# AndrewCullacino/handwritten-chinese-ocr-samples

Hardware: AMD Instinct MI355X
Metric: text-lines/sec (1x128x2000 synth) greedy decode (higher is better)
Workload: dtype f16 (f32 accumulate); 1 GPU; BASELINE configs[1]: 64 x 1x128x2000 uint8 lines, random-init hctr checkpoint (C=7358), forward + greedy CTC decode, labels to host; global_lines=64, lines_per_gpu=64, width=2000, classes=7358, checkpoint=random, parallelism=batch-shard x1

## Files before the change

### handwritten-chinese-ocr-samples_amd/csrc/engine.cpp

```cpp
#include "../../include/hctr_hip.h"
#include "kernels.h"

#include <algorithm>
#include <cfloat>
#include <cmath>
#include <cstdarg>
#include <cstdio>
#include <cstring>
#include <map>
#include <new>
#include <string>
#include <vector>

using namespace hctr;

namespace {

constexpr int kImgH = 128;
constexpr int kFeat = 2048;
constexpr double kBnEps = 1e-5;
constexpr int kStagePlanes[4] = {128, 256, 512, 512};
constexpr int kStageBlocks[4] = {2, 4, 5, 1};
constexpr int kStageH[5] = {128, 64, 32, 16, 8};
constexpr int64_t kDefaultMaxCols = 131072;
// ... 25 lines not shown
};

struct Workspace {
    int B = 0, W = 0, Wa = 0;
    void* img = nullptr;
    int32_t* widths = nullptr;
    half_t* s0 = nullptr;
    half_t* x[5] = {};
    half_t* p[5][3] = {};
    half_t* headin = nullptr;
    float* logits = nullptr;
    float* se_part = nullptr;
    float* se_scale = nullptr;
    float* se_border = nullptr;
    float* se_mean = nullptr;
    int32_t* se_counter = nullptr;
    int32_t* colidx = nullptr;
    float* amax_val = nullptr;
    int32_t* amax_idx = nullptr;
    int32_t* labels = nullptr;
    int32_t* lengths = nullptr;
    float* psum = nullptr;
    float* blank_logit = nullptr;
    float* row_thr = nullptr;
    int32_t* emit_cnt = nullptr;
    int32_t* emit_list = nullptr;
    double* esum = nullptr;
    int32_t* overflow = nullptr;
    int32_t* bm_idx = nullptr;
    float* bm_lp = nullptr;
    float* bm_bl = nullptr;
    float* bm_st = nullptr;
    int32_t* bm_cnt = nullptr;
    int32_t* tile_ctrs = nullptr;
    float* amax_val2 = nullptr;
    float* amax_abs = nullptr;
    float* col_margin = nullptr;
    float* col_abs = nullptr;
    float* line_guard = nullptr;
    int features = 0;
    bool split = false;
    bool aliased = false;
};

enum WsFeature { WS_S0 = 1, WS_LOGITS = 2, WS_BEAM = 4, WS_GUARD = 8 };

struct WeightSet {
    float* stem_w = nullptr;
    float* stem_b = nullptr;
    ConvW conv0_2;
    std::vector<BlockW> blocks[4];
    ConvW stage_conv[4];
    ConvW head;
    bool built = false;
};

struct ProfEntry {
    std::string name;
    hipEvent_t e0, e1;
};

}

struct hctr_ctx {
    int device = 0;
    int num_classes = 0;
    int cpad = 0;
    hipStream_t stream = nullptr;
    std::string err;
    std::map<std::string, HostTensor> host;
    bool finalized = false;
    WeightSet wset[2];
    const WeightSet& wts() const { return wset[split ? 1 : 0]; }
    std::vector<void*> wallocs;
    Workspace ws;
    char* arena = nullptr;
    size_t arena_cap = 0;
    int ws_sticky = 0;
    int64_t arena_reallocs = 0, ws_recarves = 0;
    int ws_alias = -1;
    size_t ws_dedicated_max = (size_t)16 << 30;
    int64_t max_cols = kDefaultMaxCols;
    bool big_tiles = true;
    int halo_mode = 2;
    int mode = 0;
    bool split = false;
    int x3_mask = 31;
    int out_class = 8;
    double guard_rel = 0.01, guard_abs = 0.05;
    std::vector<float> g_margin, g_scale;
    std::vector<uint8_t> g_flag;
    int64_t g_flagged_total = 0, g_lines_total = 0;
    std::vector<std::vector<int32_t>> h_widths;
    std::vector<int32_t> h_labels, h_lengths;
    char* pin = nullptr;
    size_t pin_cap = 0;
    int chm() const { return split ? 3 : 1; }
    bool fuse_se = true;
    std::string stamp_layer;
    unsigned long long* stamp_buf = nullptr;
    int64_t stamp_cap = 0, stamp_n = 0;
    bool fuse_ds = true;
    bool fuse_argmax = true;
    bool persist_dynamic = false;
    int conv_seq = 0;
    bool fuse_stem = true;
    bool fuse_beam = true;
    int64_t beam_fallbacks = 0;
    bool profiling = false;
    std::vector<ProfEntry> prof;
    std::vector<hipEvent_t> ev_pool;
    size_t ev_used = 0;
    std::vector<void*> beam_allocs;
    std::vector<int64_t> cand_off;
    std::vector<int32_t> cand_idx;
    std::vector<float> cand_logp;
    char* ctc_buf = nullptr;
    size_t ctc_cap = 0;
};

namespace {

int fail(hctr_ctx* c, int code, const char* fmt, ...) {
    char buf[1024];
    va_list ap;
    va_start(ap, fmt);
    vsnprintf(buf, sizeof(buf), fmt, ap);
    va_end(ap);
    if (c) c->err = buf; else g_create_error = buf;
    return code;
}

int fail_nothrow(hctr_ctx* c, int code, const char* what) noexcept {
    try {
        return fail(c, code, "%s", what);
    } catch (...) {
        return code;
    }
}

template <typename R = int, typename F>
R guard(hctr_ctx* c, F&& body) noexcept {
    try {
        return body();
    } catch (const std::bad_alloc&) {
        return (R)fail_nothrow(c, HCTR_ERR_NOMEM, "out of host memory (std::bad_alloc)");
    } catch (const std::exception& e) {
        return (R)fail_nothrow(c, HCTR_ERR_STATE, e.what());
    } catch (...) {
        return (R)fail_nothrow(c, HCTR_ERR_STATE, "unknown C++ exception");
    }
}

#define HIP_TRY(ctx, expr)                                                                        \
    do {                                                                                          \
        hipError_t _e = (expr);                                                                   \
        if (_e != hipSuccess)                                                                     \
            return fail(ctx, HCTR_ERR_HIP, "%s:%d: %s -> %s", __FILE__, __LINE__, #expr,          \
                        hipGetErrorString(_e));                                                   \
    } while (0)

#define TRY(expr)                   \
    do {                            \
        int _r = (expr);            \
        if (_r != HCTR_OK) return _r; \
    } while (0)
// ... 429 lines not shown
    if (stem_img_f32 >= 0) {
        if (tile != TILE_64x256 || cw.taps != 9 || cw.cin != 64 || cw.coutPad != 64 || c->split)
            return fail(c, HCTR_ERR_STATE, "conv %s: stem fusion not applicable", name);
        a.img = ws.img; a.img_f32 = stem_img_f32; a.img_widths = stem_widths ? ws.widths : nullptr;
        a.stem_w = c->wts().stem_w; a.stem_b = c->wts().stem_b;
        HIP_TRY(c, launch_stem_conv0_2(a, c->stream));
    } else {
        HIP_TRY(c, launch_conv(a, tile, cw.taps, false, c->stream));
    }
    pf.end();
    return HCTR_OK;
}

int run_block(hctr_ctx* c, Prof& pf, const std::string& name, const BlockW& bw, ActDesc in, half_t* t,
              half_t* o, half_t* r, int planes) {
    const Workspace& ws = c->ws;
    const int H = in.H;
    auto tiles_of = [&](const ConvW& cw) {
        const ConvTile t = pick_tile(c, cw, H);
        return (H / conv_tile_rows(t)) * ((ws.W + conv_tile_cols(t) - 1) / conv_tile_cols(t));
    };
    const float inv_hw = 1.0f / ((float)H * (float)ws.W);
    const half_t* res = in.p;
    const bool fuse_ds = bw.has_ds && c->fuse_ds && (c->fuse_se || c->split) && bw.ds.cin % kBK == 0 &&
                         pick_tile(c, bw.conv2, H) == TILE_HALO4;
    if (bw.has_ds && !fuse_ds) {
        c->out_class = 4;
        TRY(run_conv(c, pf, (name + ".downsample").c_str(), bw.ds, in, r, H, false, false, nullptr, false));
        res = r;
    }
    if (c->fuse_se || c->split) {
        const int tiles1 = tiles_of(bw.conv1);
        c->out_class = 2;
        TRY(run_conv(c, pf, (name + ".conv1").c_str(), bw.conv1, in, t, H, true, false, ws.se_part, false));
        c->out_class = 4;
        pf.begin((name + ".se_stats").c_str());
        HIP_TRY(c, launch_se_border(t, ws.B, H, ws.W, ws.Wa, planes, c->split, ws.se_part, tiles1, ws.se_border, c->stream));
        pf.end();
        pf.begin((name + ".se_scale").c_str());
        HIP_TRY(c, launch_se_premean(ws.se_border, t, bw.conv2.w, bw.conv2.bias, ws.B, H, ws.W, ws.Wa, planes,
                                     bw.conv2.coutPad, c->split, ws.se_mean, bw.se.w1, bw.se.w2, ws.se_scale,
                                     ws.se_counter, c->stream));
        pf.end();
        if (fuse_ds)
            TRY(run_conv(c, pf, (name + ".conv2+se+ds").c_str(), bw.conv2, ActDesc{t, H, planes}, o, H, true, false,
                         nullptr, false, ws.se_scale, nullptr, &bw.ds, in.p));
        else
            TRY(run_conv(c, pf, (name + ".conv2+se").c_str(), bw.conv2, ActDesc{t, H, planes}, o, H, true, false,
                         nullptr, false, ws.se_scale, res));
        return HCTR_OK;
    }
    c->out_class = 2;
    TRY(run_conv(c, pf, (name + ".conv1").c_str(), bw.conv1, in, t, H, true, false, nullptr, false));
    c->out_class = 4;
    TRY(run_conv(c, pf, (name + ".conv2").c_str(), bw.conv2, ActDesc{t, H, planes}, o, H, false, false,
                 ws.se_part, false));
    const int tiles = tiles_of(bw.conv2);
    pf.begin((name + ".se_fc").c_str());
    HIP_TRY(c, launch_se_fc(ws.se_part, tiles, bw.se.w1, bw.se.w2, ws.se_scale, ws.B, planes, inv_hw, c->stream));
    pf.end();
    pf.begin((name + ".se_apply").c_str());
    HIP_TRY(c, launch_se_apply(o, res, ws.se_scale, (int64_t)(H + 2) * ws.Wa * planes, ws.B, planes, c->stream));
    pf.end();
    return HCTR_OK;
}

enum HeadMode { HEAD_LOGITS = 0, HEAD_ARGMAX = 1, HEAD_BEAM = 2 };

int ws_need(const hctr_ctx* c, HeadMode mode, bool guarded = false) {
    int need = 0;
    if (mode == HEAD_LOGITS) need |= WS_LOGITS;
    if (mode == HEAD_BEAM) need |= WS_BEAM;
    if (!(c->fuse_stem && !c->split)) need |= WS_S0;
    if (guarded) need |= WS_GUARD;
    return need;
}

void head_args(hctr_ctx* c, ConvArgs* out, ConvTile* tile) {
    const Workspace& ws = c->ws;
    ConvArgs a{};
    a.x = ws.headin; a.w = c->wts().head.w; a.bias = c->wts().head.bias; a.y = ws.logits;
    a.Cin = c->wts().head.cin; a.Cout = c->num_classes; a.CoutPad = c->cpad;
    a.M = (int64_t)ws.B * ws.W; a.ldo = c->cpad;
    *tile = (c->big_tiles && c->cpad % 256 == 0) ? TILE_256x256 : TILE_128x128;
    const int hbm = *tile == TILE_256x256 ? 256 : 128;
    a.mtiles = (int)((a.M + hbm - 1) / hbm); a.ntiles = c->cpad / hbm;
    *out = a;
}

int run_forward(hctr_ctx* c, int img_f32, bool have_widths, HeadMode mode = HEAD_LOGITS, bool guarded = false) {
    if ((c->ws.features & ws_need(c, mode, guarded)) != ws_need(c, mode, guarded) || c->ws.split != c->split)
        return fail(c, HCTR_ERR_STATE, "workspace lacks a part this forward needs (ensure_workspace before staging)");
    Workspace& ws = c->ws;
    const WeightSet& wt = c->wts();
    if (!wt.built) return fail(c, HCTR_ERR_STATE, "the weight set of this precision mode is not resident");
    Prof pf(c);
    if (c->persist_dynamic) {
        HIP_TRY(c, hipMemsetAsync(ws.tile_ctrs, 0, 64 * 8 * 4, c->stream));
        c->conv_seq = 0;
    }
    auto zero_stage = [&](int s, bool input, bool blocks) -> int {
        if (!ws.aliased) return HCTR_OK;
        const int H = kStageH[s], planes = kStagePlanes[s - 1], cin_s = s == 1 ? 64 : kStagePlanes[s - 2];
        const int mm = c->chm();
        pf.begin("zero_borders");
        if (input) HIP_TRY(c, launch_zero_borders(ws.x[s], ws.B, H, ws.W, ws.Wa, cin_s * mm, c->stream));
        for (int i = 0; blocks && i < ((s == 4) ? 2 : 3); ++i)
            HIP_TRY(c, launch_zero_borders(ws.p[s][i], ws.B, H, ws.W, ws.Wa, planes * mm, c->stream));
        pf.end();
        return HCTR_OK;
    };
    TRY(zero_stage(1, true, true));
    c->out_class = 8;
    if (c->fuse_stem && !c->split) {
        TRY(run_conv(c, pf, "stem+conv0_2+pool", wt.conv0_2, ActDesc{nullptr, 128, 64}, ws.x[1], 64, true, true, nullptr,
                     false, nullptr, nullptr, nullptr, nullptr, img_f32 ? 1 : 0, have_widths));
    } else {
        pf.begin("stem.conv0_1");
        HIP_TRY(c, launch_stem(ws.img, img_f32, have_widths ? ws.widths : nullptr, wt.stem_w, wt.stem_b, ws.s0, ws.B,
                               ws.W, ws.Wa, c->split ? ((c->x3_mask & 8) ? 1 : 2) : 0, c->stream));
        pf.end();
        TRY(run_conv(c, pf, "conv0_2+pool", wt.conv0_2, ActDesc{ws.s0, 128, 64}, ws.x[1], 64, true, true, nullptr, false));
    }
    int cin = 64;
    for (int s = 1; s <= 4; ++s) {
        const int H = kStageH[s], planes = kStagePlanes[s - 1];
        ActDesc cur{ws.x[s], H, cin};
        int ci = -1;
        for (size_t i = 0; i < wt.blocks[s - 1].size(); ++i) {
            const BlockW& bw = wt.blocks[s - 1][i];
            char nm[48];
            snprintf(nm, sizeof(nm), "block%d.%zu", s, i);
            const int ti = ci < 0 ? 0 : (ci + 1) % 3, oi = ci < 0 ? 1 : (ci + 2) % 3;
            if (bw.has_ds && ci >= 0) return fail(c, HCTR_ERR_STATE, "downsample only expected on a stage's first block");
            TRY(run_block(c, pf, nm, bw, cur, ws.p[s][ti], ws.p[s][oi], bw.has_ds ? ws.p[s][2] : nullptr, planes));
            cur = ActDesc{ws.p[s][oi], H, planes};
            ci = oi;
        }
        char nm[32];
        snprintf(nm, sizeof(nm), "conv%d+pool", s);
        c->out_class = s < 4 ? 8 : 16;
        if (s < 4) {
            TRY(zero_stage(s + 1, true, false));
            TRY(run_conv(c, pf, nm, wt.stage_conv[s - 1], cur, ws.x[s + 1], H / 2, true, true, nullptr, false));
            TRY(zero_stage(s + 1, false, true));
        } else
            TRY(run_conv(c, pf, nm, wt.stage_conv[s - 1], cur, ws.headin, H / 2, true, true, nullptr, true));
        cin = planes;
    }
    ConvArgs a;
    ConvTile htile;
    head_args(c, &a, &htile);
    auto line_guard = [&]() -> int {
        pf.begin("line_guard");
        HIP_TRY(c, launch_line_guard(ws.col_margin, ws.col_abs, ws.B, ws.W, ws.line_guard, c->stream));
        pf.end();
        return HCTR_OK;
    };
    if (mode == HEAD_ARGMAX || mode == HEAD_BEAM) {
        a.y = nullptr;
        a.amax_val = ws.amax_val;
        a.amax_idx = ws.amax_idx;
        if (guarded) { a.amax_val2 = ws.amax_val2; a.amax_abs = ws.amax_abs; }
        if (mode == HEAD_BEAM) { a.psum = ws.psum; a.blank_logit = ws.blank_logit; }
        pf.begin(mode == HEAD_BEAM ? "head.linear+partials" : "head.linear+argmax");
        HIP_TRY(c, launch_conv(a, htile, 1, true, c->stream));
// ... 360 lines not shown
                                   c->stream));
    pf.end();
    const size_t co = (size_t)b0 * W, cb = n * W * 4;
    auto fetch = [&](void* dst, const void* src, size_t bytes) {
        return dst ? hipMemcpyAsync(dst, src, bytes, hipMemcpyDeviceToHost, c->stream) : hipSuccess;
    };
    HIP_TRY(c, fetch(h_lab ? h_lab + co : nullptr, d_lab, cb));
    HIP_TRY(c, fetch(h_len ? h_len + b0 : nullptr, d_len, n * 4));
    HIP_TRY(c, fetch(o.span_start ? o.span_start + co : nullptr, d_st, cb));
    HIP_TRY(c, fetch(o.span_end ? o.span_end + co : nullptr, d_en, cb));
    HIP_TRY(c, fetch(o.char_logp ? o.char_logp + co : nullptr, d_clp, cb));
    HIP_TRY(c, fetch(o.alt_label ? o.alt_label + co : nullptr, d_alab, cb));
    HIP_TRY(c, fetch(o.alt_logp ? o.alt_logp + co : nullptr, d_alp, cb));
    HIP_TRY(c, fetch(o.path_logp ? o.path_logp + b0 : nullptr, d_plp, n * 4));
    if (!o.text_nll) return HCTR_OK;
    std::vector<float> plp(n);
    HIP_TRY(c, fetch(plp.data(), d_plp, n * 4));
    HIP_TRY(c, hipStreamSynchronize(c->stream));
    std::vector<int32_t> tg, tl((size_t)nb);
    for (int b = 0; b < nb; ++b) {
        const int L = h_len[b0 + b];
        const bool fits = 2 * (int64_t)L + 1 <= kCtcMaxStates;
        tl[(size_t)b] = fits ? L : 0;
        if (fits) tg.insert(tg.end(), h_lab + (co + (size_t)b * W), h_lab + (co + (size_t)b * W) + L);
    }
    CtcHost h;
    TRY(ctc_prepare(c, nb, W, C, tg.data(), tl.data(), nullptr, &h));
    const size_t tab_b = align256(h.tab.size() * 4);
    TRY(ctc_reserve(c, lse_b + tab_b + line_b + n * W * h.D * 4, lse_b));
    d_lse = (double*)c->ctc_buf;
    const CtcLines m = h.lines((const int32_t*)(c->ctc_buf + lse_b));
    float* d_nll = (float*)(c->ctc_buf + lse_b + tab_b);
    float* emis = (float*)(c->ctc_buf + lse_b + tab_b + line_b);
    HIP_TRY(c, hipMemcpyAsync(c->ctc_buf + lse_b, h.tab.data(), h.tab.size() * 4, hipMemcpyHostToDevice, c->stream));
    pf.begin("ctc_emis_gather");
    HIP_TRY(c, launch_ctc_emis_gather(x, ld, sb, st, m, 0, nb, W, d_lse, emis, c->stream));
    pf.end();
    pf.begin("ctc_alpha");
    HIP_TRY(c, launch_ctc_alpha(emis, m, 0, nb, W, h.max_states, d_nll, nullptr, nullptr, c->stream));
    pf.end();
    HIP_TRY(c, hipMemcpyAsync(o.text_nll + b0, d_nll, n * 4, hipMemcpyDeviceToHost, c->stream));
    HIP_TRY(c, hipStreamSynchronize(c->stream));
    for (int b = 0; b < nb; ++b)
        if (tl[(size_t)b] != h_len[b0 + b] || plp[(size_t)b] != plp[(size_t)b])
            o.text_nll[b0 + b] = std::numeric_limits<float>::quiet_NaN();
    return HCTR_OK;
}

}

extern "C" {

#ifndef HCTR_SRC_HASH
#define HCTR_SRC_HASH "unhashed-build000"
#endif
const char* hctr_version(void) {
    return "hctr-hip 0.3 (gfx950, f16 storage / f16 MFMA / f32 accumulate; f16x3 split precision; guarded mode) "
           "hctr-src=" HCTR_SRC_HASH;
}

int hctr_create(hctr_ctx** out, int device, int num_classes) {
    return guard(nullptr, [&]() -> int {
        if (!out) return fail(nullptr, HCTR_ERR_ARG, "out is NULL");
        *out = nullptr;
        if (num_classes < 3) return fail(nullptr, HCTR_ERR_ARG, "num_classes must be >= 3 (blank + chars + unknown)");
        int ndev = 0;
        hipError_t e = hipGetDeviceCount(&ndev);
        if (e != hipSuccess || ndev == 0)
            return fail(nullptr, HCTR_ERR_HIP, "no HIP device available (%s): the hctr engine has no CPU fallback",
                        hipGetErrorString(e));
        if (device < 0 || device >= ndev) return fail(nullptr, HCTR_ERR_ARG, "device %d out of range [0,%d)", device, ndev);
        e = hipSetDevice(device);
        if (e != hipSuccess) return fail(nullptr, HCTR_ERR_HIP, "hipSetDevice(%d): %s", device, hipGetErrorString(e));
        hctr_ctx* c = new hctr_ctx();
        c->device = device;
        c->num_classes = num_classes;
        c->cpad = (num_classes + 255) / 256 * 256;
        e = hipStreamCreateWithFlags(&c->stream, hipStreamNonBlocking);
        if (e != hipSuccess) {
            delete c;
            return fail(nullptr, HCTR_ERR_HIP, "hipStreamCreate: %s", hipGetErrorString(e));
        }
        if (const char* bt = getenv("HCTR_BIG_TILES")) c->big_tiles = atoi(bt) != 0;
        if (const char* hm = getenv("HCTR_HALO")) c->halo_mode = atoi(hm);
        if (const char* pr = getenv("HCTR_PRECISION")) {
            const std::string m(pr);
            c->mode = m == "f16x3" ? 1 : (m == "auto" ? 2 : 0);
            c->split = c->mode == 1;
        }
        if (const char* fs = getenv("HCTR_FUSE_SE")) c->fuse_se = atoi(fs) != 0;
        if (const char* fa = getenv("HCTR_FUSE_ARGMAX")) c->fuse_argmax = atoi(fa) != 0;
        if (const char* fd = getenv("HCTR_FUSE_DS")) c->fuse_ds = atoi(fd) != 0;
        if (const char* fb = getenv("HCTR_FUSE_BEAM")) c->fuse_beam = atoi(fb) != 0;
        if (const char* fs2 = getenv("HCTR_FUSE_STEM")) c->fuse_stem = atoi(fs2) != 0;
        if (const char* ps = getenv("HCTR_PERSIST")) c->persist_dynamic = atoi(ps) == 2;
        if (const char* xm = getenv("HCTR_X3_MASK")) c->x3_mask = atoi(xm) & 31;
        if (const char* wa = getenv("HCTR_WS_ALIAS")) c->ws_alias = atoi(wa) != 0 ? 1 : 0;
        if (const char* wd = getenv("HCTR_WS_DEDICATED_MAX_GB")) {
            const double g = atof(wd);
            if (g >= 0) c->ws_dedicated_max = (size_t)(g * 1073741824.0);
        }
        if (const char* mc = getenv("HCTR_MAX_COLS")) {
            const long long v = atoll(mc);
            if (v > 0) c->max_cols = v;
        }
        *out = c;
        return HCTR_OK;
    });
}

void hctr_destroy(hctr_ctx* c) {
    if (!c) return;
    (void)hipSetDevice(c->device);
    (void)hipStreamSynchronize(c->stream);
    if (c->arena) (void)hipFree(c->arena);
    if (c->pin) (void)hipHostFree(c->pin);
    free_pool(c->wallocs);
    free_pool(c->beam_allocs);
    if (c->ctc_buf) (void)hipFree(c->ctc_buf);
    if (c->stamp_buf) (void)hipFree(c->stamp_buf);
    for (hipEvent_t e : c->ev_pool) (void)hipEventDestroy(e);
    (void)hipStreamDestroy(c->stream);
    delete c;
}

const char* hctr_last_error(const hctr_ctx* c) { return c ? c->err.c_str() : g_create_error.c_str(); }

int hctr_load_tensor(hctr_ctx* c, const char* key, const void* host_ptr, const int64_t* shape, int ndim, int dtype) {
    return guard(c, [&]() -> int {
        if (!c) return HCTR_ERR_ARG;
        if (!key || (!host_ptr && ndim > 0) || ndim < 0 || ndim > 8) return fail(c, HCTR_ERR_ARG, "bad tensor arguments");
        if (c->finalized) return fail(c, HCTR_ERR_STATE, "weights already finalized");
        const std::string k(key);
        if (dtype == HCTR_I64) {
            if (k.size() < 19 || k.compare(k.size() - 19, 19, "num_batches_tracked") != 0)
                return fail(c, HCTR_ERR_KEY, "Unexpected key(s) in state_dict: \"%s\" (int64)", key);
            return HCTR_OK;
        }
        if (dtype != HCTR_F32) return fail(c, HCTR_ERR_ARG, "tensor %s: only float32 parameters are supported", key);
        HostTensor t;
        int64_t n = 1;
        for (int i = 0; i < ndim; ++i) {
            if (shape[i] < 0) return fail(c, HCTR_ERR_ARG, "negative dimension");
            t.shape.push_back(shape[i]);
            n *= shape[i];
        }
        t.data.assign((const float*)host_ptr, (const float*)host_ptr + n);
        c->host[k] = std::move(t);
        return HCTR_OK;
    });
}

int hctr_finalize_weights(hctr_ctx* c) {
    return guard(c, [&]() -> int {
        if (!c) return HCTR_ERR_ARG;
        if (c->finalized) return fail(c, HCTR_ERR_STATE, "weights already finalized");
        HIP_TRY(c, hipSetDevice(c->device));
        auto build_set = [&](bool split) -> int {
            c->split = split;
            WeightSet& ws = c->wset[split ? 1 : 0];
            TRY(build_stem(c, ws));
            TRY(build_conv(c, "cnn.conv0_2", "cnn.bn0_2", 64, 64, 3, true, 64, &ws.conv0_2));
            int inpl = 64;
            for (int s = 0; s < 4; ++s) {
                const int planes = kStagePlanes[s];
                ws.blocks[s].assign(kStageBlocks[s], BlockW());
// ... 914 lines not shown
```

### handwritten-chinese-ocr-samples_amd/csrc/kernels.h

```cpp
#pragma once
#include <hip/hip_runtime.h>
#include <stdint.h>

namespace hctr {

typedef _Float16 half_t;

constexpr int kTileW = 16;
constexpr int kBK = 64;

struct ConvArgs {
    const half_t* x;
    const half_t* w;
    const float* bias;
    void* y;
    float* se_part;
    const float* se_scale;
    const half_t* resid;
    int H, W;
    int Cin, Cout, CoutPad;
    int tilesW, tilesH;
    int64_t in_sb;
    int in_sh;
    int64_t out_sb;
    int out_sh, out_sw;
    int64_t out_off;
    int out_wlimit;
    int relu, pool;
    int64_t M;
    int64_t ldo;
    int mtiles, ntiles;
    int nt_shift, th_shift;
    uint64_t tw_magic;
    float* amax_val;
    int32_t* amax_idx;
    float* amax_val2;
    float* amax_abs;
    float* psum;
    float* blank_logit;
    const float* row_thr;
    int32_t* emit_cnt;
    int32_t* emit_list;
    int emit_cap;
    double* esum;
    const void* img;
    int img_f32;
    const int32_t* img_widths;
    const float* stem_w;
    const float* stem_b;
    int split;
    int drop_lo;
    const half_t* ds_x;
    const half_t* ds_w;
    const float* ds_bias;
    int ds_cin;
    int ds_in_sh;
    int64_t ds_in_sb;
    int32_t* tile_counter;
    unsigned long long* stamps;
    int dbg;
};

enum ConvTile { TILE_64x256 = 0, TILE_128x128 = 1, TILE_256x256 = 2, TILE_HALO4 = 3, TILE_HALO4_8x32 = 4 };
inline int conv_tile_rows(ConvTile t) { return (t == TILE_128x128 || t == TILE_HALO4_8x32) ? 8 : 16; }
inline int conv_tile_cols(ConvTile t) { return t == TILE_HALO4_8x32 ? 32 : 16; }
inline int conv_tile_couts(ConvTile t) {
    return t == TILE_64x256 ? 64 : (t == TILE_256x256 ? 256 : 128);
}

hipError_t launch_conv(const ConvArgs& a, ConvTile tile, int taps, bool linear_f32, hipStream_t s);
constexpr int kLinearWN = 2;
hipError_t launch_argmax_partials(const float* val, const int32_t* cls, int P, int64_t M, int32_t* idx, hipStream_t s,
                                  const float* val2 = nullptr, const float* absp = nullptr, float* margin = nullptr,
                                  float* rowabs = nullptr);
hipError_t launch_row_guard(const float* logits, int64_t ld, int64_t M, int C, float* margin, float* rowabs, hipStream_t s);
hipError_t launch_line_guard(const float* margin, const float* rowabs, int B, int W, float* out, hipStream_t s);
size_t conv_lds_bytes(ConvTile tile);

hipError_t launch_stem_conv0_2(const ConvArgs& a, hipStream_t s);

hipError_t launch_zero_borders(half_t* p, int B, int H, int W, int Wa, int C, hipStream_t s);

hipError_t launch_stem(const void* img, int img_f32, const int32_t* widths_dev, const float* w9,
                       const float* bias, half_t* y, int B, int W, int Wa, int split, hipStream_t s);

hipError_t launch_se_border(const half_t* t, int B, int H, int W, int Wa, int C, int split, const float* tsum_part,
                            int tiles, float* out, hipStream_t s);
hipError_t launch_se_premean(const float* border, const half_t* t, const half_t* w, const float* bias, int B, int H,
                             int W, int Wa, int C, int CoutPad, int split, float* mean, const float* w1,
                             const float* w2, float* scale, int32_t* counter, hipStream_t s);

hipError_t launch_se_fc(const float* se_part, int tiles_per_img, const float* w1, const float* w2,
                        float* scale, int B, int C, float inv_hw, hipStream_t s);

hipError_t launch_se_apply(half_t* o, const half_t* r, const float* scale, int64_t img_elems,
                           int B, int C, hipStream_t s);

hipError_t launch_argmax_rows(const float* logits, int64_t ld, int64_t M, int C, int32_t* idx,
                              int tB, int tW, hipStream_t s);

constexpr int kBeamCap = 256;
constexpr int kBeamMaxK = 32;
hipError_t launch_beam_thresholds(const float* pmax, const float* psum, int P, int64_t M, int k, double cand_thresh,
                                  int want_candidates, float* row_thr, int32_t* emit_cnt, hipStream_t s);
hipError_t launch_beam_select(const float* row_thr, const int32_t* emit_cnt, const int32_t* emit_list, int cap,
                              const double* esum, int P, const float* blank_logit, int B, int W, int k,
                              double cand_thresh, int32_t* topk_idx, float* topk_logp, float* blank_logp,
                              float* stats, int32_t* cand_count, int32_t* overflow, hipStream_t s);
hipError_t launch_beam_candidates(const int32_t* emit_cnt, const int32_t* emit_list, int cap, const float* stats,
                                  int B, int W, double cand_thresh, const int64_t* cand_off, int32_t* cand_idx,
                                  float* cand_logp, hipStream_t s);

hipError_t launch_ctc_collapse(const int32_t* idx, int B, int W, int C, int32_t* labels,
// ... 66 lines not shown
```

### handwritten-chinese-ocr-samples_amd/csrc/kernels.hip

```cpp
#include "kernels.h"

#include <algorithm>
#include <cstdlib>

namespace hctr {

typedef _Float16 f16x8 __attribute__((ext_vector_type(8)));
typedef float f32x4 __attribute__((ext_vector_type(4)));
typedef float f32x2 __attribute__((ext_vector_type(2)));
typedef _Float16 f16x2 __attribute__((ext_vector_type(2)));
typedef uint32_t u32x4 __attribute__((ext_vector_type(4)));
typedef void __attribute__((address_space(3))) * lptr_t;

__device__ __forceinline__ void glds16_asm(const char* gsrc, char* lds_dst) {
    const uint32_t lds = (uint32_t)(uintptr_t)((lptr_t)lds_dst);
    uint32_t keep;
    asm volatile("s_mov_b32 %0, m0\n\ts_mov_b32 m0, %2\n\ts_nop 0\n\tglobal_load_lds_dwordx4 %1, off\n\ts_mov_b32 m0, %0"
                 : "=&s"(keep)
                 : "v"(gsrc), "s"(lds)
                 : "memory");
}

template <int CTRL>
__device__ __forceinline__ float dpp_f32(float v) {
// ... 565 lines not shown
                read_b(0, bq[0]);
                read_a(0, ar[0]);
                __builtin_amdgcn_sched_barrier(0);
                read_a(1, ar[1]);
                __builtin_amdgcn_sched_barrier(0);
                if (k + 1 < nk) stage(k + 1, (k + 1) & 1);
                __builtin_amdgcn_sched_barrier(0);
#pragma unroll
                for (int g = 0; g < 8; ++g) {
                    if (g + 2 < 8) read_a(g + 2, ar[(g + 2) % 3]);
                    __builtin_amdgcn_sched_barrier(0);
                    if (g == 1) { read_b(1, bq[1]); __builtin_amdgcn_sched_barrier(0); }
                    __builtin_amdgcn_s_setprio(1);
#pragma unroll
                    for (int jj = 0; jj < 2; ++jj)
#pragma unroll
                        for (int n = 0; n < 4; ++n)
                            acc[2 * (g & 3) + jj][n] = __builtin_amdgcn_mfma_f32_16x16x32_f16(ar[g % 3][jj], bq[g >> 2][n],
                                                                                             acc[2 * (g & 3) + jj][n], 0, 0, 0);
                    __builtin_amdgcn_s_setprio(0);
                    __builtin_amdgcn_sched_barrier(0);
                }
                continue;
            }
            if (k + 1 < nk) stage(k + 1, (k + 1) & 1);
#pragma unroll
            for (int ks = 0; ks < 2; ++ks) {
                const int fo = ks ? foff1 : foff0;
                f16x8 af[JT], bf[4];
#pragma unroll
                for (int n = 0; n < 4; ++n) bf[n] = *(const f16x8*)(xt + n * 2048 + fo);
#pragma unroll
                for (int j = 0; j < JT; ++j) af[j] = *(const f16x8*)(wt + j * 2048 + fo);
                __builtin_amdgcn_s_setprio(1);
#pragma unroll
                for (int j = 0; j < JT; ++j)
#pragma unroll
                    for (int n = 0; n < 4; ++n)
                        acc[j][n] = __builtin_amdgcn_mfma_f32_16x16x32_f16(af[j], bf[n], acc[j][n], 0, 0, 0);
                __builtin_amdgcn_s_setprio(0);
            }
        }
    } else {
        constexpr int NG = 2 * JT;
        constexpr int NP = NIW + NIX;
        for (int k = 0; k < nk; ++k) {
            asm volatile("s_waitcnt vmcnt(0)" ::: "memory");
            __syncthreads();
            const int kn = k + 1 < nk ? k + 1 : k;
            int64_t wo_n, xo_n;
            step_offsets(kn, wo_n, xo_n);
            const char* wsrc_n = wbase + wo_n;
            const char* xsrc_n = xbase + xo_n;
            const int buf_n = (k + 1) & 1;
            const char* wt = smem + (k & 1) * TILE_BYTES + (wn * WC) * 128;
            const char* xt = smem + (k & 1) * TILE_BYTES + BN * 128 + (wm * 64) * 128;
            f16x8 bfr[2][4], afr[2];
#pragma unroll
            for (int n = 0; n < 4; ++n) bfr[0][n] = *(const f16x8*)(xt + n * 2048 + foff0);
            afr[0] = *(const f16x8*)(wt + foff0);
#pragma unroll
            for (int g = 0; g < NG; ++g) {
                const int ks = g / JT, j = g % JT;
                if (g + 1 < NG) {
                    const int ks1 = (g + 1) / JT, j1 = (g + 1) % JT;
                    afr[(g + 1) & 1] = *(const f16x8*)(wt + j1 * 2048 + (ks1 ? foff1 : foff0));
                }
                if (g == JT / 2) {
#pragma unroll
                    for (int n = 0; n < 4; ++n) bfr[1][n] = *(const f16x8*)(xt + n * 2048 + foff1);
                }
                if ((g * NP) / NG != ((g + 1) * NP) / NG)
                    stage_piece(wsrc_n, xsrc_n, buf_n, (g * NP) / NG);
#pragma unroll
                for (int n = 0; n < 4; ++n)
                    acc[j][n] = __builtin_amdgcn_mfma_f32_16x16x32_f16(afr[g & 1], bfr[ks][n], acc[j][n], 0, 0, 0);
                __builtin_amdgcn_sched_barrier(0);
            }
        }
    }

    conv_epilogue<WN, WM, JT, LINEAR, SPLIT>(a, acc, smem, tid, lane, wn, wm, n0, mt, img, th, tw,
                                             th * (4 * WM) + wm * 4, tw * kTileW);
}

static int env_dbg() {
    if (getenv("HCTR_DBG_LAYER")) return 0;
    const char* e = getenv("HCTR_DBG");
    return e ? atoi(e) : 0;
}

static hipError_t raise_lds_limit(const void* fn, int bytes, bool (&done)[64]) {
    int dev = 0;
    hipError_t e = hipGetDevice(&dev);
    if (e != hipSuccess) return e;
    if (dev < 0 || dev >= 64) return hipErrorInvalidDevice;
    if (done[dev]) return hipSuccess;
    e = hipFuncSetAttribute(fn, hipFuncAttributeMaxDynamicSharedMemorySize, bytes);
    if (e == hipSuccess) done[dev] = true;
    return e;
}

constexpr int kHaloCols = 20;
constexpr int kHaloRows = 18;
constexpr int kHaloBytes = kHaloRows * kHaloCols * 128;
constexpr int kHaloPieces = kHaloRows * kHaloCols / 8;
constexpr int kHaloLds = 2 * 32768 + 2 * kHaloBytes;

__global__ __launch_bounds__(512) void conv3x3_halo_kernel(const ConvArgs a) {
    constexpr int WN = 2, WM = 4, JT = 8, BN = 256;
    extern __shared__ __attribute__((aligned(16))) char smem[];
    const int tid = threadIdx.x;
    const int lane = tid & 63;
    const int wv = __builtin_amdgcn_readfirstlane(tid >> 6);
    const int wn = wv / WM, wm = wv % WM;

    const int total = a.mtiles * a.ntiles;
    int lin;
    {
        const int id = blockIdx.x, xcd = id & 7, s = id >> 3;
        const int q = total >> 3, r = total & 7;
        lin = (xcd < r ? xcd * (q + 1) : r * (q + 1) + (xcd - r) * q) + s;
    }
    const int nt = lin % a.ntiles;
    const int mt = lin / a.ntiles;
    const int n0 = nt * BN;
    const int tw = mt % a.tilesW;
    const int t2 = mt / a.tilesW;
    const int th = t2 % a.tilesH;
    const int img = t2 / a.tilesH;
    const int cin = a.Cin;
    const int nkc = cin / kBK;

    const char* xbase = (const char*)(a.x + img * a.in_sb + (int64_t)(th * 16) * a.in_sh + (int64_t)(tw * 16) * cin);
    const char* wbase = (const char*)(a.w + (int64_t)n0 * cin);
    const bool loader = wv < 4;
    uint32_t woff[8], hoff[12];
#pragma unroll
    for (int i = 0; i < 8; ++i) {
        const int g = ((wv & 3) * 8 + i) * 64 + lane;
        const int row = g >> 3, cp = (g & 7) ^ (row & 7);
        woff[i] = (uint32_t)row * (uint32_t)cin * 2u + cp * 16;
    }
#pragma unroll
    for (int r = 0; r < 12; ++r) {
        const int piece = ((r >> 1) * 4 + (wv & 3)) * 2 + (r & 1);
        const int g = piece * 64 + lane;
        const int row = g >> 3, cp = (g & 7) ^ (row & 7);
        int hy = row / kHaloCols, hx = row - hy * kHaloCols;
        if (hx > 17) hx = 17;
        if (hy > 17) hy = 17;
        hoff[r] = ((uint32_t)hy * (uint32_t)a.in_sh + (uint32_t)hx * (uint32_t)cin) * 2u + cp * 16;
    }
    const int q = lane >> 4, c = lane & 15;
    const int aoff0 = c * 128 + (((0 + q) ^ (lane & 7)) << 4);
    const int aoff1 = c * 128 + (((4 + q) ^ (lane & 7)) << 4);

    auto stage_weights = [&](int kc, int tap, int buf) {
        const char* src = wbase + ((int64_t)tap * a.CoutPad * cin + (int64_t)kc * kBK) * 2;
        char* dst = smem + buf * 32768 + ((wv & 3) * 8) * 1024;
#pragma unroll
        for (int i = 0; i < 8; ++i)
            glds16_asm(src + woff[i], dst + i * 1024);
    };
    auto stage_halo_piece = [&](int kc, int buf, int piece, uint32_t off) {
        if (piece < kHaloPieces) {
// ... 698 lines not shown
        if (dev >= 0 && dev < 64 && cus[dev] == 0) {
            hipDeviceProp_t prop;
            if (hipGetDeviceProperties(&prop, dev) == hipSuccess) cus[dev] = prop.multiProcessorCount;
            if (cus[dev] <= 0) cus[dev] = 256;
        }
        const int resident = 2 * ((dev >= 0 && dev < 64) ? cus[dev] : 256);
        if (grid > resident) grid = resident;
        grid = (grid + 7) / 8 * 8;
    }
    return launch_halo4_instance<conv3x3_halo4_kernel<GEOM, SPLIT, PERSIST>>(a, grid, s);
}
template <int GEOM, bool SPLIT>
static hipError_t launch_conv_halo4_t(const ConvArgs& a, hipStream_t s) {
    const int grid = a.mtiles * a.ntiles;
    if (a.ds_x != nullptr) {
        if (GEOM != 0) return hipErrorInvalidValue;
        return launch_halo4_instance<conv3x3_halo4_kernel<0, SPLIT, false, false, true>>(a, grid, s);
    }
    if (a.stamps != nullptr && !SPLIT)
        return launch_halo4_instance<conv3x3_halo4_kernel<GEOM, false, false, true>>(a, grid, s, false);
    static const int persist = [] { const char* e = getenv("HCTR_PERSIST"); return e ? atoi(e) : 0; }();
    if constexpr (!SPLIT) {
        static const int respre = [] { const char* e = getenv("HCTR_RESPRE"); return e ? atoi(e) : 0; }();
        if (respre && persist == 0 && a.resid != nullptr && a.se_scale != nullptr)
            return launch_halo4_instance<conv3x3_halo4_kernel<GEOM, false, false, false, false, true>>(a, grid, s);
    }
    if (persist == 0 || (persist == 2 && a.tile_counter == nullptr)) return launch_conv_halo4_tp<GEOM, SPLIT, false>(a, s);
    ConvArgs b = a;
    if (persist != 2) b.tile_counter = nullptr;
    return launch_conv_halo4_tp<GEOM, SPLIT, true>(b, s);
}
template <int GEOM>
static hipError_t launch_conv_halo4(const ConvArgs& a0, hipStream_t s) {
    ConvArgs a = a0;
    auto shift_of = [](int v) { int sft = 0; while ((1 << sft) < v) ++sft; return (1 << sft) == v ? sft : -1; };
    a.nt_shift = shift_of(a.ntiles);
    a.th_shift = shift_of(a.tilesH);
    if (a.tilesW < 1 || (uint64_t)a.mtiles * (uint64_t)a.tilesW >= ((uint64_t)1 << 40)) return hipErrorInvalidValue;
    a.tw_magic = (((uint64_t)1 << 40) + (uint64_t)a.tilesW - 1) / (uint64_t)a.tilesW;
    static const bool halfhalo = [] { const char* e = getenv("HCTR_HALFHALO"); return e ? atoi(e) != 0 : false; }();
    static const int persist = [] { const char* e = getenv("HCTR_PERSIST"); return e ? atoi(e) : 0; }();
    if (halfhalo && !a.split && a.ds_x == nullptr && a.stamps == nullptr && persist == 0 && a.Cin % kBK == 0)
        return launch_halo4_instance<conv3x3_halo4h_kernel<GEOM>>(a, a.mtiles * a.ntiles, s);
    return a.split ? launch_conv_halo4_t<GEOM, true>(a, s) : launch_conv_halo4_t<GEOM, false>(a, s);
}

static hipError_t launch_conv_halo(const ConvArgs& a, hipStream_t s) {
    static bool done[64] = {};
    hipError_t e0 = raise_lds_limit((const void*)conv3x3_halo_kernel, kHaloLds, done);
    if (e0 != hipSuccess) return e0;
    static const int dbg = env_dbg();
    ConvArgs b = a;
    b.dbg |= dbg;
    hipLaunchKernelGGL(conv3x3_halo_kernel, dim3(a.mtiles * a.ntiles), dim3(512), kHaloLds, s, b);
    return hipGetLastError();
}

size_t conv_lds_bytes(ConvTile tile) {
    switch (tile) {
        case TILE_64x256: return 2 * (64 + 256) * 128;
        case TILE_256x256: return 2 * (256 + 256) * 128;
        default: return 2 * (128 + 128) * 128;
    }
}

template <int WN, int WM, int JT, int TAPS, bool LINEAR, bool PIPE, bool SPLIT>
static hipError_t launch_conv_ts(const ConvArgs& a, size_t lds, hipStream_t s) {
    auto kern = conv_mfma_kernel<WN, WM, JT, TAPS, LINEAR, PIPE, SPLIT>;
    static bool done[64] = {};
    hipError_t e0 = raise_lds_limit((const void*)kern, (int)lds, done);
    if (e0 != hipSuccess) return e0;
    const int grid = a.mtiles * a.ntiles;
    hipLaunchKernelGGL(kern, dim3(grid), dim3(WN * WM * 64), lds, s, a);
    return hipGetLastError();
}
template <int WN, int WM, int JT, int TAPS, bool LINEAR, bool PIPE>
static hipError_t launch_conv_t(const ConvArgs& a, size_t lds, hipStream_t s) {
    if constexpr (!LINEAR && !PIPE) {
        if (a.split) return launch_conv_ts<WN, WM, JT, TAPS, LINEAR, PIPE, true>(a, lds, s);
    }
    return launch_conv_ts<WN, WM, JT, TAPS, LINEAR, PIPE, false>(a, lds, s);
}

hipError_t launch_conv(const ConvArgs& a, ConvTile tile, int taps, bool linear_f32, hipStream_t s) {
    const size_t lds = conv_lds_bytes(tile);
    static const int halo = [] { const char* e = getenv("HCTR_HALO"); return e ? atoi(e) : 2; }();
    static const bool pipe = [] { const char* e = getenv("HCTR_PIPE"); return e ? atoi(e) != 0 : false; }();
    if (linear_f32) {
        if (tile == TILE_256x256)
            return pipe ? launch_conv_t<2, 4, 8, 1, true, true>(a, lds, s) : launch_conv_t<2, 4, 8, 1, true, false>(a, lds, s);
        return launch_conv_t<2, 2, 4, 1, true, false>(a, lds, s);
    }
    switch (tile) {
        case TILE_HALO4:
            return taps == 9 ? launch_conv_halo4<0>(a, s) : hipErrorInvalidValue;
        case TILE_HALO4_8x32:
            return taps == 9 ? launch_conv_halo4<1>(a, s) : hipErrorInvalidValue;
        case TILE_64x256:
            return taps == 9 ? launch_conv_t<1, 4, 4, 9, false, false>(a, lds, s)
                             : launch_conv_t<1, 4, 4, 1, false, false>(a, lds, s);
        case TILE_256x256:
            if (taps == 9 && halo) return launch_conv_halo(a, s);
            if (taps == 9)
                return pipe ? launch_conv_t<2, 4, 8, 9, false, true>(a, lds, s)
                            : launch_conv_t<2, 4, 8, 9, false, false>(a, lds, s);
            return launch_conv_t<2, 4, 8, 1, false, false>(a, lds, s);
        default:
            return taps == 9 ? launch_conv_t<2, 2, 4, 9, false, false>(a, lds, s)
                             : launch_conv_t<2, 2, 4, 1, false, false>(a, lds, s);
    }
}

constexpr int kStemRows = 16;

__global__ __launch_bounds__(256) void stem_kernel(const void* __restrict__ img, int img_f32,
                                                   const int32_t* __restrict__ widths,
                                                   const float* __restrict__ w9,
                                                   const float* __restrict__ bias,
                                                   half_t* __restrict__ y, int B, int W, int Wa, int split) {
    const int cg = threadIdx.x & 7;
    const int w = blockIdx.x * 32 + (threadIdx.x >> 3);
    const int h0 = blockIdx.y * kStemRows;
    const int b = blockIdx.z;
    if (w >= W) return;
    float wt[8][9], bs[8];
#pragma unroll
    for (int e = 0; e < 8; ++e) {
        bs[e] = bias[cg * 8 + e];
#pragma unroll
        for (int t = 0; t < 9; ++t) wt[e][t] = w9[(cg * 8 + e) * 9 + t];
    }
    const int wlim = widths ? widths[b] : W;
    auto pixel = [&](int hh, int ww) -> float {
        if (hh < 0 || hh >= 128 || ww < 0 || ww >= W) return 0.f;
        const int wsrc = ww < wlim ? ww : wlim - 1;
        const int64_t off = ((int64_t)b * 128 + hh) * W + wsrc;
        if (img_f32) return ((const float*)img)[off];
        float x = (float)((const uint8_t*)img)[off] / 255.0f;
        return (x - 0.5f) / 0.5f;
    };
    float win[3][3];
#pragma unroll
    for (int r = 0; r < 2; ++r)
#pragma unroll
        for (int d = 0; d < 3; ++d) win[r + 1][d] = pixel(h0 - 1 + r, w - 1 + d);
    const int cs = split ? 192 : 64;
    for (int r = 0; r < kStemRows; ++r) {
        const int h = h0 + r;
#pragma unroll
        for (int d = 0; d < 3; ++d) {
            win[0][d] = win[1][d];
            win[1][d] = win[2][d];
            win[2][d] = pixel(h + 1, w - 1 + d);
        }
        f16x8 o, ol;
#pragma unroll
        for (int e = 0; e < 8; ++e) {
            float sv = bs[e];
#pragma unroll
            for (int t = 0; t < 9; ++t) sv = fmaf(wt[e][t], win[t / 3][t % 3], sv);
            sv = fmaxf(sv, 0.f);
            o[e] = (half_t)sv;
            ol[e] = split == 2 ? (half_t)0.f : (half_t)(sv - (float)o[e]);
        }
        half_t* dst = y + (((int64_t)b * 130 + h + 1) * Wa + (w + 1)) * cs + cg * 8;
        *(f16x8*)dst = o;
        if (split) {
            *(f16x8*)(dst + 64) = ol;
            *(f16x8*)(dst + 128) = o;
        }
    }
// ... 1762 lines not shown
```

Measured before the change: 519.5 lines/s.

## Add ping-pong double-buffered MFMA kernel for the linear head GEMM

Adds a dedicated head GEMM kernel that double-buffers K tiles in LDS and staggers two groups of waves with barriers so one group issues global-to-LDS loads while the other runs MFMAs, using s_setprio to favour the math phase. It also remaps block IDs across the eight XCDs so contiguous tiles land on the same XCD. It is enabled by default for the 256x256 linear head when HCTR_PIPE is off. The cost targeted is exposed load latency in the large-vocabulary classifier GEMM. The risks are more LDS usage and fragile barrier pairing between the wave groups.

```diff
diff --git a/handwritten-chinese-ocr-samples_amd/csrc/engine.cpp b/handwritten-chinese-ocr-samples_amd/csrc/engine.cpp
--- a/handwritten-chinese-ocr-samples_amd/csrc/engine.cpp
+++ b/handwritten-chinese-ocr-samples_amd/csrc/engine.cpp
@@ -131,6 +131,7 @@
     size_t ws_dedicated_max = (size_t)16 << 30;
     int64_t max_cols = kDefaultMaxCols;
     bool big_tiles = true;
+    bool head_pp = true;
     int halo_mode = 2;
     int mode = 0;
     bool split = false;
@@ -726,6 +727,7 @@
     a.x = ws.headin; a.w = c->wts().head.w; a.bias = c->wts().head.bias; a.y = ws.logits;
     a.Cin = c->wts().head.cin; a.Cout = c->num_classes; a.CoutPad = c->cpad;
     a.M = (int64_t)ws.B * ws.W; a.ldo = c->cpad;
+    a.head_pp = c->head_pp ? 1 : 0;
     *tile = (c->big_tiles && c->cpad % 256 == 0) ? TILE_256x256 : TILE_128x128;
     const int hbm = *tile == TILE_256x256 ? 256 : 128;
     a.mtiles = (int)((a.M + hbm - 1) / hbm); a.ntiles = c->cpad / hbm;
@@ -1252,6 +1254,7 @@
             return fail(nullptr, HCTR_ERR_HIP, "hipStreamCreate: %s", hipGetErrorString(e));
         }
         if (const char* bt = getenv("HCTR_BIG_TILES")) c->big_tiles = atoi(bt) != 0;
+        if (const char* hp = getenv("HCTR_HEAD_PP")) c->head_pp = atoi(hp) != 0;
         if (const char* hm = getenv("HCTR_HALO")) c->halo_mode = atoi(hm);
         if (const char* pr = getenv("HCTR_PRECISION")) {
             const std::string m(pr);
diff --git a/handwritten-chinese-ocr-samples_amd/csrc/kernels.h b/handwritten-chinese-ocr-samples_amd/csrc/kernels.h
--- a/handwritten-chinese-ocr-samples_amd/csrc/kernels.h
+++ b/handwritten-chinese-ocr-samples_amd/csrc/kernels.h
@@ -29,6 +29,7 @@
     int relu, pool;
     int64_t M;
     int64_t ldo;
+    int head_pp;
     int mtiles, ntiles;
     int nt_shift, th_shift;
     uint64_t tw_magic;
diff --git a/handwritten-chinese-ocr-samples_amd/csrc/kernels.hip b/handwritten-chinese-ocr-samples_amd/csrc/kernels.hip
--- a/handwritten-chinese-ocr-samples_amd/csrc/kernels.hip
+++ b/handwritten-chinese-ocr-samples_amd/csrc/kernels.hip
@@ -671,6 +671,110 @@
 
     conv_epilogue<WN, WM, JT, LINEAR, SPLIT>(a, acc, smem, tid, lane, wn, wm, n0, mt, img, th, tw,
                                              th * (4 * WM) + wm * 4, tw * kTileW);
+}
+
+__global__ __launch_bounds__(512) void head_gemm_pp_kernel(const ConvArgs a) {
+    constexpr int WN = kLinearWN, WM = 4, JT = 8;
+    constexpr int WC = JT * 16, BN = WN * WC, BM = WM * 64;
+    constexpr int TILE_BYTES = (BN + BM) * 128;
+    extern __shared__ __attribute__((aligned(16))) char smem[];
+
+    const int tid = threadIdx.x;
+    const int lane = tid & 63;
+    const int wv = __builtin_amdgcn_readfirstlane(tid >> 6);
+    const int grp = wv >> 2, wr = wv & 3;
+    const int wm = grp * 2 + (wr >> 1), wn = wr & 1;
+
+    const int total = a.mtiles * a.ntiles;
+    int lin;
+    {
+        const int id = blockIdx.x, xcd = id & 7, s = id >> 3;
+        const int q = total >> 3, r = total & 7;
+        lin = (xcd < r ? xcd * (q + 1) : r * (q + 1) + (xcd - r) * q) + s;
+    }
+    const int nt = lin % a.ntiles;
+    const int mt = lin / a.ntiles;
+    const int n0 = nt * BN;
+    const int cin = a.Cin;
+
+    const char* xbase = (const char*)(a.x + (int64_t)mt * BM * cin);
+    const char* wbase = (const char*)(a.w + (int64_t)n0 * cin) + (int64_t)(wr * 64) * cin * 2;
+    uint32_t xoff[4];
+    {
+        const int64_t rem = a.M - (int64_t)mt * BM;
+#pragma unroll
+        for (int i = 0; i < 4; ++i) {
+            const int row = (wv * 4 + i) * 8 + (lane >> 3), cp = (lane & 7) ^ (row & 7);
+            const int r = (int64_t)row < rem ? row : (int)rem - 1;
+            xoff[i] = (uint32_t)r * (uint32_t)cin * 2u + cp * 16;
+        }
+    }
+    const uint32_t woff = (uint32_t)(lane >> 3) * (uint32_t)cin * 2u + (((lane & 7) ^ (lane >> 3)) << 4);
+    const int64_t wpiece = (int64_t)cin * 16;
+    auto stage = [&](int k, int buf) {
+        const int64_t ko = (int64_t)k * (kBK * 2);
+        char* dst = smem + buf * TILE_BYTES;
+        if (grp == 0) {
+            const char* ws = wbase + ko;
+            char* wd = dst + wr * 8192;
+            glds16x4_asm_s(ws, ws + wpiece, ws + 2 * wpiece, ws + 3 * wpiece, woff, wd, wd + 1024, wd + 2048, wd + 3072);
+            glds16x4_asm_s(ws + 4 * wpiece, ws + 5 * wpiece, ws + 6 * wpiece, ws + 7 * wpiece, woff, wd + 4096, wd + 5120,
+                           wd + 6144, wd + 7168);
+        }
+        glds16x4v_asm_s<1024>(xbase + ko, xoff[0], xoff[1], xoff[2], xoff[3], dst + BN * 128 + wv * 4096);
+    };
+
+    f32x4 acc[JT][4];
+#pragma unroll
+    for (int j = 0; j < JT; ++j)
+#pragma unroll
+        for (int n = 0; n < 4; ++n) acc[j][n] = (f32x4){0.f, 0.f, 0.f, 0.f};
+
+    const int q = lane >> 4;
+    const int frow = lane & 15;
+    const int foff0 = frow * 128 + (((0 + q) ^ (lane & 7)) << 4);
+    const int foff1 = frow * 128 + (((4 + q) ^ (lane & 7)) << 4);
+    const int nk = cin / kBK;
+
+    stage(0, 0);
+    asm volatile("s_waitcnt vmcnt(0)" ::: "memory");
+    __builtin_amdgcn_s_barrier();
+    if (grp == 1) __builtin_amdgcn_s_barrier();
+    for (int k = 0; k < nk; ++k) {
+        const char* wt = smem + (k & 1) * TILE_BYTES + (wn * WC) * 128;
+        const char* xt = smem + (k & 1) * TILE_BYTES + BN * 128 + (wm * 64) * 128;
+        __builtin_amdgcn_sched_barrier(0);
+        if (k + 1 < nk) stage(k + 1, (k + 1) & 1);
+        __builtin_amdgcn_sched_barrier(0);
+        f16x8 af[2][JT], bf[2][4];
+#pragma unroll
+        for (int ks = 0; ks < 2; ++ks) {
+            const int fo = ks ? foff1 : foff0;
+#pragma unroll
+            for (int n = 0; n < 4; ++n) bf[ks][n] = *(const f16x8*)(xt + n * 2048 + fo);
+#pragma unroll
+            for (int j = 0; j < JT; ++j) af[ks][j] = *(const f16x8*)(wt + j * 2048 + fo);
+        }
+        __builtin_amdgcn_sched_barrier(0);
+        asm volatile("s_waitcnt lgkmcnt(0)" ::: "memory");
+        __builtin_amdgcn_s_barrier();
+        __builtin_amdgcn_sched_barrier(0);
+        __builtin_amdgcn_s_setprio(1);
+#pragma unroll
+        for (int ks = 0; ks < 2; ++ks)
+#pragma unroll
+            for (int j = 0; j < JT; ++j)
+#pragma unroll
+                for (int n = 0; n < 4; ++n)
+                    acc[j][n] = __builtin_amdgcn_mfma_f32_16x16x32_f16(af[ks][j], bf[ks][n], acc[j][n], 0, 0, 0);
+        __builtin_amdgcn_s_setprio(0);
+        __builtin_amdgcn_sched_barrier(0);
+        asm volatile("s_waitcnt vmcnt(0)" ::: "memory");
+        __builtin_amdgcn_s_barrier();
+    }
+    if (grp == 0) __builtin_amdgcn_s_barrier();
+
+    conv_epilogue<WN, WM, JT, true, false>(a, acc, smem, tid, lane, wn, wm, n0, mt, 0, 0, 0, 0, 0);
 }
 
 static int env_dbg() {
@@ -1535,11 +1639,20 @@
     return launch_conv_ts<WN, WM, JT, TAPS, LINEAR, PIPE, false>(a, lds, s);
 }
 
+static hipError_t launch_head_pp(const ConvArgs& a, size_t lds, hipStream_t s) {
+    static bool done[64] = {};
+    hipError_t e0 = raise_lds_limit((const void*)head_gemm_pp_kernel, (int)lds, done);
+    if (e0 != hipSuccess) return e0;
+    hipLaunchKernelGGL(head_gemm_pp_kernel, dim3(a.mtiles * a.ntiles), dim3(512), lds, s, a);
+    return hipGetLastError();
+}
+
 hipError_t launch_conv(const ConvArgs& a, ConvTile tile, int taps, bool linear_f32, hipStream_t s) {
     const size_t lds = conv_lds_bytes(tile);
     static const int halo = [] { const char* e = getenv("HCTR_HALO"); return e ? atoi(e) : 2; }();
     static const bool pipe = [] { const char* e = getenv("HCTR_PIPE"); return e ? atoi(e) != 0 : false; }();
     if (linear_f32) {
+        if (tile == TILE_256x256 && a.head_pp && !pipe) return launch_head_pp(a, lds, s);
         if (tile == TILE_256x256)
             return pipe ? launch_conv_t<2, 4, 8, 1, true, true>(a, lds, s) : launch_conv_t<2, 4, 8, 1, true, false>(a, lds, s);
         return launch_conv_t<2, 2, 4, 1, true, false>(a, lds, s);
```

Measured after the change: 520.7 lines/s (median of 6 runs). No clear change (+0.2%).
